# manhtuando97/two-stage-gnn

Hardware: NVIDIA B200
Metric: train graphs/sec (fwd+bwd) (higher is better)
Workload: dtype f32

## Files before the change

### include/tsg.h

```cpp
#ifndef TSG_H_
#define TSG_H_

#include <stddef.h>
#include <stdint.h>

#ifdef __cplusplus
extern "C" {
#endif

#define TSG_ABI_VERSION 1

enum {
  TSG_OK = 0,
  TSG_EINVAL = -1,
  TSG_EWORKSPACE = -2,
  TSG_ELAUNCH = -3,
  TSG_EARCH = -4
};

int tsg_abi_version(void);
const char* tsg_last_error(void);
int tsg_check_device(void);
int tsg_init_device(void);

// ... 190 lines not shown
int tsg_linkpred_loss_fwd(const float* S, const int64_t* graph_ptr, const int32_t* rowptr, const int32_t* colidx,
                          int64_t num_graphs, int64_t assign_dim, double num_entries, float eps, float* loss,
                          void* workspace, size_t workspace_bytes, void* stream);
int tsg_linkpred_loss_bwd(const float* S, const int64_t* graph_ptr, const int32_t* rowptr, const int32_t* colidx,
                          int64_t num_graphs, int64_t assign_dim, double num_entries, float eps, const float* dloss,
                          float* dS, void* stream);

#define TSG_TU_NETWORKX 0
#define TSG_TU_PYG 1
typedef struct tsg_tu_handle tsg_tu_handle;
int tsg_tu_load(const char* prefix, int mode, int64_t max_nodes , tsg_tu_handle** out);
int tsg_tu_sizes(const tsg_tu_handle* h, int64_t* sizes);
int tsg_tu_fill(const tsg_tu_handle* h, int64_t* node_ptr, int64_t* edge_ptr, int64_t* row, int64_t* col,
                int32_t* node_label, int64_t* y, float* attr );
void tsg_tu_free(tsg_tu_handle* h);

int tsg_csr_build_graphs_sym_local(const int32_t* local_row, const int32_t* local_col, const int64_t* edge_ptr,
                                   const int64_t* node_ptr, int64_t num_graphs, int64_t num_nodes, int64_t num_edges,
                                   int64_t max_graph_nodes, int32_t* rowptr, int32_t* colidx, float* val,
                                   int32_t* status, void* stream);

typedef struct {
  int64_t num_graphs, in_feat, hidden, num_edges;
  int64_t n[4];
  int64_t max_graph_nodes[3];
  int64_t max_graph_edges;
  double pooling_ratio;
  int64_t flags;
  int32_t* status;
} tsg_sag_shape;
#define TSG_SAG_COALESCED 1
size_t tsg_sag_arena_bytes(const tsg_sag_shape* shape);
int tsg_sag_set_fused(int on);
enum { TSG_SAG_PERM = 0, TSG_SAG_SCORE = 1, TSG_SAG_H = 2, TSG_SAG_XG = 3, TSG_SAG_ROWPTR = 4, TSG_SAG_COLIDX = 5,
       TSG_SAG_VAL = 6, TSG_SAG_INV = 7, TSG_SAG_STATUS = 8  };
int tsg_sag_arena_locate(const tsg_sag_shape* shape, int level, int field, size_t* offset, size_t* bytes);
int tsg_sag_encoder_fwd(const tsg_sag_shape* shape, const float* x, const int64_t* row, const int64_t* col,
                        const int64_t* level_ptr, const float* const* params, float* z,
                        void* arena, size_t arena_bytes, void* stream);
int tsg_sag_encoder_bwd(const tsg_sag_shape* shape, const float* x, const int64_t* level_ptr,
                        const float* const* params, const float* dz, float* const* grads,
                        void* arena, size_t arena_bytes, void* stream);

typedef struct {
  int64_t num_classes;
  int64_t num_triplets;
  float margin, eps, dropout_p;
  uint64_t seed;
} tsg_sag_head;
size_t tsg_sag_triplet_step_workspace_bytes(const tsg_sag_shape* shape, const tsg_sag_head* head);
int tsg_sag_triplet_step_compact(const tsg_sag_shape* shape, const tsg_sag_head* head, const int32_t* label,
                                 const int32_t* local_row, const int32_t* local_col, const int64_t* edge_ptr,
                                 const int64_t* level_ptr, const float* const* params, const int64_t* triplets,
                                 const float* dropout_mask , float* const* grads, float* loss,
                                 float* emb_out , void* arena, size_t arena_bytes, void* workspace,
                                 size_t workspace_bytes, void* stream);

int tsg_sag_step_fwd_compact(const tsg_sag_shape* shape, const tsg_sag_head* head, const int32_t* label,
                             const int32_t* local_row, const int32_t* local_col, const int64_t* edge_ptr,
                             const int64_t* level_ptr, const float* const* params, const float* dropout_mask ,
                             float* emb, void* arena, size_t arena_bytes, void* workspace, size_t workspace_bytes,
                             void* stream);
int tsg_sag_step_bwd_compact(const tsg_sag_shape* shape, const tsg_sag_head* head, const int32_t* label,
                             const int64_t* level_ptr, const float* const* params, const float* emb, const float* demb,
                             float* const* grads, void* arena, size_t arena_bytes, void* workspace,
                             size_t workspace_bytes, void* stream);
// ... 50 lines not shown
```

### two-stage-gnn_b200/csrc/k10_sag_exec.cu

```cuda
#include "common.cuh"
#include "sag_fused.cuh"

namespace tsg {

struct LevelBuf {
  int64_t* eptr;
  int32_t *rowptr, *colidx, *t_rowptr, *t_colidx;
  float *val, *t_val;
  float *xw, *h, *sw, *score, *xg, *out;
  int64_t* perm;
  int32_t* inv;
  int32_t* argmax;
};

struct SagArena {
  LevelBuf lv[3];
  float *dxg, *dh, *dhm, *dxw, *dscore, *dsw;
  void* scratch; size_t scratch_bytes;
  unsigned* sched; int* status;
  size_t total;
};

static size_t scratch_need(const tsg_sag_shape* sh) {
  size_t m = 0;
  auto up = [&](size_t v) { if (v > m) m = v; };
  for (int l = 0; l < 3; ++l) {
    up(tsg_csr_build_graphs_workspace_bytes(sh->num_graphs, sh->num_edges));
    up(tsg_topk_workspace_bytes(sh->n[l], sh->num_graphs));
    up(tsg_csr_filter_workspace_bytes(sh->n[l + 1]));
    up(2 * tsg_colsum_workspace_bytes(sh->n[l], sh->hidden));
    up(tsg_linear_bwd_weight_workspace_bytes(l == 0 ? sh->in_feat : sh->hidden, sh->hidden));
    up(tsg_linear_bwd_weight_workspace_bytes(sh->hidden, 1));
  }
  up(tsg_embed_bwd_weight_workspace_bytes(sh->in_feat, sh->hidden));
  up(tsg_gate_score_bwd_workspace_bytes());
  return align_up(m, 256) + 256;
}

static void layout(const tsg_sag_shape* sh, void* arena, SagArena* a) {
  char* base = (char*)arena;
  size_t off = 0;
  auto take = [&](size_t bytes) -> void* {
    void* p = base ? (void*)(base + off) : nullptr;
    off += align_up(bytes, 256);
    return p;
  };
  const int64_t G = sh->num_graphs, H = sh->hidden, E = sh->num_edges;
  for (int l = 0; l < 3; ++l) {
    LevelBuf& b = a->lv[l];
    const int64_t n = sh->n[l], k = sh->n[l + 1], cap = E + n;
    b.eptr = (int64_t*)take((G + 1) * 8);
    b.rowptr = (int32_t*)take((n + 1) * 4); b.t_rowptr = (int32_t*)take((n + 1) * 4);
    b.colidx = (int32_t*)take(cap * 4); b.t_colidx = (int32_t*)take(cap * 4);
    b.val = (float*)take(cap * 4); b.t_val = (float*)take(cap * 4);
    b.xw = (float*)take(n * H * 4); b.h = (float*)take(n * H * 4);
    b.sw = (float*)take(n * 4); b.score = (float*)take(n * 4);
    b.perm = (int64_t*)take((k > 0 ? k : 1) * 8);
    b.inv = (int32_t*)take((n > 0 ? n : 1) * 4);
    b.xg = (float*)take((k > 0 ? k : 1) * H * 4);
    b.out = (float*)take(G * 2 * H * 4);
    b.argmax = (int32_t*)take(G * H * 4);
  }
  const int64_t n0 = sh->n[0] > 0 ? sh->n[0] : 1;
  a->dxg = (float*)take(n0 * H * 4); a->dh = (float*)take(n0 * H * 4);
  a->dhm = (float*)take(n0 * H * 4); a->dxw = (float*)take(n0 * H * 4);
  a->dscore = (float*)take(n0 * 4); a->dsw = (float*)take(n0 * 4);
// ... 5 lines not shown
  a->total = off;
  if (sh->flags & TSG_SAG_COALESCED)
    for (int l = 0; l < 3; ++l) {
      LevelBuf& b = a->lv[l];
      b.t_rowptr = b.rowptr; b.t_colidx = b.colidx; b.t_val = b.val;
    }
}

__global__ void __launch_bounds__(256)
k_add3(const float* __restrict__ a, const float* __restrict__ b, const float* __restrict__ c, float* __restrict__ o, int64_t n) {
  for (int64_t i = (int64_t)blockIdx.x * blockDim.x + threadIdx.x; i < n; i += (int64_t)gridDim.x * blockDim.x)
    o[i] = (a[i] + b[i]) + c[i];
}

struct SagInput {
  const float* x;
  const int64_t *row, *col;
  const int32_t* label;
  const int32_t *lrow, *lcol;
  const int64_t* edge_ptr;
};

static bool sag_unfused_env() {
  static const bool v = getenv("TSG_SAG_UNFUSED") != nullptr;
  return v;
}

static int g_sag_fused = -1;
static bool sag_fused_env() {
  if (g_sag_fused < 0) g_sag_fused = !(getenv("TSG_SAG_FUSED") && getenv("TSG_SAG_FUSED")[0] == '0');
  return g_sag_fused != 0;
}

static bool use_fused(const tsg_sag_shape* sh, bool compact) {
  if (!compact || !sag_fused_env() || sh->max_graph_edges <= 0) return false;
  for (int l = 0; l < 3; ++l) if (sh->max_graph_nodes[l] > 32767) return false;
  return fused_supported((int)sh->hidden, (int)sh->in_feat, (int)sh->max_graph_nodes[0], (int)sh->max_graph_nodes[1],
                         (int)sh->max_graph_edges);
}

static void fill_fused(FusedArgs& f, const tsg_sag_shape* sh, const SagArena& a, const int32_t* label, const int32_t* lrow,
                       const int32_t* lcol, const int64_t* edge_ptr, const int64_t* level_ptr, const float* const* params) {
  f.G = (int)sh->num_graphs; f.L = (int)sh->in_feat; f.H = (int)sh->hidden;
  for (int l = 0; l < 3; ++l) f.nmax[l] = (int)sh->max_graph_nodes[l];
  f.emax = (int)sh->max_graph_edges;
  f.ratio = (float)sh->pooling_ratio; f.avg_degree = (double)sh->num_edges / (double)(sh->n[0] > 0 ? sh->n[0] : 1);
  f.cls = 0; f.cls_nlo = 0; f.cls_elo = -1;
  f.label = label; f.lrow = lrow; f.lcol = lcol; f.edge_ptr = edge_ptr; f.level_ptr = level_ptr;
  for (int i = 0; i < 12; ++i) f.params[i] = params[i];
  for (int l = 0; l < 3; ++l) {
    f.h[l] = a.lv[l].h; f.score[l] = a.lv[l].score; f.perm[l] = a.lv[l].perm; f.argmax[l] = a.lv[l].argmax;
  }
  f.z = nullptr;
  f.sched = a.sched; f.status = a.status;
}

static bool shape_ok(const tsg_sag_shape* sh) {
  if (!sh || sh->num_graphs <= 0 || sh->in_feat <= 0 || sh->hidden <= 0 || sh->num_edges < 0) return false;
  for (int l = 0; l < 4; ++l) if (sh->n[l] <= 0) return false;
  for (int l = 0; l < 3; ++l) if (sh->max_graph_nodes[l] <= 0) return false;
  return true;
}

}

using namespace tsg;

#define TSG_TRY(call)                 \
  do {                                \
    int _rc = (call);                 \
    if (_rc != TSG_OK) return _rc;    \
  } while (0)

extern "C" int tsg_sag_set_fused(int on) {
  const int prev = sag_fused_env() ? 1 : 0;
  g_sag_fused = on ? 1 : 0;
  return prev;
}

extern "C" size_t tsg_sag_arena_bytes(const tsg_sag_shape* shape) {
  if (!shape_ok(shape)) return 0;
  SagArena a;
  layout(shape, nullptr, &a);
  return a.total;
}

extern "C" int tsg_sag_arena_locate(const tsg_sag_shape* sh, int level, int field, size_t* offset, size_t* bytes) {
  TSG_REQUIRE(shape_ok(sh) && level >= 0 && level < 3 && offset && bytes, "sag_arena_locate: bad argument");
  SagArena a;
  char* const base = (char*)256;
  tsg_sag_shape own = *sh;
  own.status = nullptr;
  layout(&own, base, &a);
  const LevelBuf& b = a.lv[level];
  const int64_t n = sh->n[level], k = sh->n[level + 1], H = sh->hidden;
  const void* p = nullptr; size_t sz = 0;
  switch (field) {
    case TSG_SAG_PERM: p = b.perm; sz = (size_t)k * 8; break;
    case TSG_SAG_SCORE: p = b.score; sz = (size_t)n * 4; break;
    case TSG_SAG_H: p = b.h; sz = (size_t)n * H * 4; break;
    case TSG_SAG_XG: p = b.xg; sz = (size_t)k * H * 4; break;
    case TSG_SAG_ROWPTR: p = b.rowptr; sz = (size_t)(n + 1) * 4; break;
    case TSG_SAG_COLIDX: p = b.colidx; sz = (size_t)(sh->num_edges + n) * 4; break;
    case TSG_SAG_VAL: p = b.val; sz = (size_t)(sh->num_edges + n) * 4; break;
    case TSG_SAG_INV: p = b.inv; sz = (size_t)n * 4; break;
    case TSG_SAG_STATUS: p = a.status; sz = 4; break;
    default: set_error("sag_arena_locate: unknown field %d", field); return TSG_EINVAL;
  }
  *offset = (size_t)((const char*)p - base);
  *bytes = sz;
  return TSG_OK;
}

static int sag_fwd(const tsg_sag_shape* sh, const SagInput& in, const int64_t* level_ptr, const float* const* params,
                   float* z, void* arena, size_t arena_bytes, void* stream, bool forward_only = false) {
  SagArena a;
  layout(sh, arena, &a);
  if (arena_bytes < a.total) { set_error("sag_encoder_fwd: arena too small (%zu < %zu)", arena_bytes, a.total); return TSG_EWORKSPACE; }
  cudaStream_t st = (cudaStream_t)stream;
  const int64_t G = sh->num_graphs, H = sh->hidden, E = sh->num_edges;
  if (!sh->status) cudaMemsetAsync(a.status, 0, sizeof(int), st);
  if (forward_only && use_fused(sh, in.label != nullptr)) {
    FusedArgs f;
    fill_fused(f, sh, a, in.label, in.lrow, in.lcol, in.edge_ptr, level_ptr, params);
    f.z = z;
    return launch_sag_fused_fwd(f, st);
  }
  const float* xin = in.x;
  bool xw_ready = false;
  for (int l = 0; l < 3; ++l) {
    LevelBuf& b = a.lv[l];
    const int64_t n = sh->n[l], k = sh->n[l + 1], fin = l == 0 ? sh->in_feat : H;
    const float *W = params[4 * l], *bias = params[4 * l + 1], *ws = params[4 * l + 2], *bs = params[4 * l + 3];
    const int64_t* ptr_l = level_ptr + (size_t)l * (G + 1);
    const int64_t* ptr_n = level_ptr + (size_t)(l + 1) * (G + 1);
    const bool sym = in.label && (sh->flags & TSG_SAG_COALESCED);
    if (l == 0 && sym) {
      TSG_TRY(tsg_csr_build_graphs_sym_local(in.lrow, in.lcol, in.edge_ptr, ptr_l, G, n, E, sh->max_graph_nodes[l], b.rowptr,
                                             b.colidx, b.val, a.status, stream));
    } else if (l == 0 && in.label) {
      TSG_TRY(tsg_csr_build_graphs_local(in.lrow, in.lcol, in.edge_ptr, ptr_l, G, n, E, sh->max_graph_nodes[l], b.rowptr,
                                         b.colidx, b.val, nullptr, b.t_rowptr, b.t_colidx, b.t_val, nullptr, a.scratch,
                                         a.scratch_bytes, stream));
    } else if (l == 0) {
      TSG_TRY(tsg_edge_ptr(in.row, E, nullptr, ptr_l, G, b.eptr, stream));
      TSG_TRY(tsg_csr_build_graphs(in.row, in.col, b.eptr, ptr_l, G, n, E, sh->max_graph_nodes[l], b.rowptr, b.colidx, b.val,
                                   nullptr, b.t_rowptr, b.t_colidx, b.t_val, nullptr, a.scratch, a.scratch_bytes, stream));
    } else {
      const LevelBuf& pb = a.lv[l - 1];
      if (sym) TSG_TRY(tsg_csr_filter(pb.rowptr, pb.colidx, nullptr, nullptr, pb.perm, pb.inv, n, b.rowptr, b.colidx, b.val,
                                      nullptr, nullptr, nullptr, a.scratch, a.scratch_bytes, stream));
      else TSG_TRY(tsg_csr_filter(pb.rowptr, pb.colidx, pb.t_rowptr, pb.t_colidx, pb.perm, pb.inv, n, b.rowptr, b.colidx, b.val,
                                  b.t_rowptr, b.t_colidx, b.t_val, a.scratch, a.scratch_bytes, stream));
    }
    static const bool no_label_spmm = getenv("TSG_NO_LABEL_SPMM") != nullptr;
    const bool label_spmm = l == 0 && in.label && H % 4 == 0 && H <= 128 && !no_label_spmm &&
                            ((((uintptr_t)W) | ((uintptr_t)bias) | ((uintptr_t)ws)) & 15) == 0;
    if (label_spmm) {
      TSG_TRY(tsg_spmm_label_dot(b.rowptr, b.colidx, b.val, W, in.label, fin, bias, b.h, ws, b.sw, n, H, TSG_SPMM_RELU, stream));
    } else {
      if (l == 0 && in.label) TSG_TRY(tsg_embed_fwd(W, in.label, b.xw, n, fin, H, stream));
      else if (!xw_ready) TSG_TRY(tsg_linear_fwd(xin, W, nullptr, b.xw, n, fin, H, 0, 0, stream));
      TSG_TRY(tsg_spmm_dot(b.rowptr, b.colidx, b.val, b.xw, bias, b.h, ws, b.sw, n, H, TSG_SPMM_RELU, stream));
    }
    TSG_TRY(tsg_spmm(b.rowptr, b.colidx, b.val, b.sw, bs, b.score, n, 1, 0, stream));
    TSG_TRY(tsg_topk_bounded(b.score, ptr_l, ptr_n, G, n, sh->max_graph_nodes[l], b.perm, a.scratch, a.scratch_bytes, stream));
    TSG_TRY(tsg_inv_perm(b.perm, k, n, b.inv, stream));
    static const bool no_gr = getenv("TSG_NO_GATE_READOUT") != nullptr;
    if (H % 4 == 0 && !sag_unfused_env() && !no_gr) {
      const bool next_xw = l < 2 && (((uintptr_t)params[4 * (l + 1)]) & 15) == 0;
      TSG_TRY(tsg_gate_readout_linear_fwd(b.h, b.score, b.perm, ptr_n, G, k, H, b.xg, b.out, 2 * H, b.argmax,
                                          next_xw ? params[4 * (l + 1)] : nullptr, next_xw ? a.lv[l + 1].xw : nullptr, stream));
      xw_ready = next_xw;
    } else {
      xw_ready = false;
      TSG_TRY(tsg_gate_gather_fwd(b.h, b.score, b.perm, nullptr, b.xg, nullptr, k, H, stream));
      TSG_TRY(tsg_readout_fwd(b.xg, ptr_n, G, H, TSG_READOUT_MAX | TSG_READOUT_MEAN, b.out, 2 * H, b.argmax, stream));
    }
    xin = b.xg;
  }
  const int64_t tot = G * 2 * H;
  k_add3<<<grid_for(tot, 256, 8), 256, 0, st>>>(a.lv[0].out, a.lv[1].out, a.lv[2].out, z, tot);
  return check_launch("sag_encoder_fwd");
}

extern "C" int tsg_sag_encoder_fwd(const tsg_sag_shape* sh, const float* x, const int64_t* row, const int64_t* col,
                                   const int64_t* level_ptr, const float* const* params, float* z,
                                   void* arena, size_t arena_bytes, void* stream) {
  TSG_REQUIRE(shape_ok(sh), "sag_encoder_fwd: bad shape");
  TSG_REQUIRE(x && level_ptr && params && z && arena && (sh->num_edges == 0 || (row && col)), "sag_encoder_fwd: null pointer");
  const SagInput in{x, row, col, nullptr, nullptr, nullptr, nullptr};
  return sag_fwd(sh, in, level_ptr, params, z, arena, arena_bytes, stream);
}

extern "C" int tsg_sag_encoder_fwd_compact(const tsg_sag_shape* sh, const int32_t* label, const int32_t* local_row,
                                           const int32_t* local_col, const int64_t* edge_ptr, const int64_t* level_ptr,
                                           const float* const* params, float* z, void* arena, size_t arena_bytes,
                                           void* stream) {
  TSG_REQUIRE(shape_ok(sh), "sag_encoder_fwd_compact: bad shape");
  TSG_REQUIRE(label && edge_ptr && level_ptr && params && z && arena && (sh->num_edges == 0 || (local_row && local_col)),
// ... 79 lines not shown
```

### two-stage-gnn_b200/csrc/k5_topk.cu

```cuda
#include "common.cuh"
#include <stdlib.h>

namespace tsg {

__device__ __forceinline__ uint32_t score_key(float s) {
  if (s != s) return 0xFFFFFFFFu;
  if (s == 0.f) s = 0.f;
  uint32_t b = __float_as_uint(s);
  return (b & 0x80000000u) ? ~b : (b | 0x80000000u);
}

struct KofN {
  const int64_t* gptr; float ratio;
  __device__ int operator()(int64_t g) const {
    float n = (float)(gptr[g + 1] - gptr[g]);
    return (int)ceilf(__fmul_rn(ratio, n));
  }
};

constexpr int TOPK_THREADS = 128;
constexpr int TOPK_SMEM_KEYS = 4096;

__global__ void __launch_bounds__(TOPK_THREADS)
k_topk_rank(const float* __restrict__ score, const int64_t* __restrict__ gptr,
            const int64_t* __restrict__ kptr, int64_t* __restrict__ perm, unsigned long long* __restrict__ gkeys,
            int skip_upto) {
  __shared__ __align__(16) unsigned long long skeys[TOPK_SMEM_KEYS];
  const int g = blockIdx.x;
  const int64_t base = gptr[g];
  const int n = (int)(gptr[g + 1] - base);
  const int64_t obase = kptr[g];
  const int k = (int)(kptr[g + 1] - obase);
  if (n == 0 || k == 0) return;
  if (n <= skip_upto) return;
  const bool in_smem = n <= TOPK_SMEM_KEYS;
  unsigned long long* keys = in_smem ? skeys : (gkeys + base);
  for (int i = threadIdx.x; i < n; i += TOPK_THREADS)
    keys[i] = ((unsigned long long)score_key(score[base + i]) << 32) | (unsigned long long)(0xFFFFFFFFu - (unsigned)i);
  __syncthreads();
  for (int i = threadIdx.x; i < n; i += TOPK_THREADS) {
    const unsigned long long ki = keys[i];
    int rank = 0;
    int j = 0;
// ... 12 lines not shown
            int64_t* __restrict__ perm, int max_pad, int min_n) {
  extern __shared__ __align__(16) unsigned long long sk[];
  {
    const int g = blockIdx.x;
    const int64_t base = gptr[g];
    const int n = (int)(gptr[g + 1] - base);
    const int64_t obase = kptr[g];
    const int k = (int)(kptr[g + 1] - obase);
    if (n == 0 || k == 0) return;
    if (n > max_pad) return;
    if (n <= min_n) return;
    int npad = 32; while (npad < n) npad <<= 1;
    for (int i = threadIdx.x; i < npad; i += TOPK_SORT_THREADS)
      sk[i] = i < n ? (((unsigned long long)score_key(score[base + i]) << 32) | (unsigned long long)(0xFFFFFFFFu - (unsigned)i)) : 0ull;
    __syncthreads();
    for (int kk = 2; kk <= npad; kk <<= 1) {
      for (int j = kk >> 1; j > 0; j >>= 1) {
        for (int t = threadIdx.x; t < (npad >> 1); t += TOPK_SORT_THREADS) {
          const int i = ((t & ~(j - 1)) << 1) | (t & (j - 1));
          const int l = i | j;
          const unsigned long long a = sk[i], b = sk[l];
          const bool desc = (i & kk) == 0;
          if ((a < b) == desc) { sk[i] = b; sk[l] = a; }
        }
        __syncthreads();
      }
    }
    for (int i = threadIdx.x; i < k; i += TOPK_SORT_THREADS)
      perm[obase + i] = base + (int64_t)(0xFFFFFFFFu - (unsigned)(sk[i] & 0xFFFFFFFFull));
  }
}


constexpr int TOPK_RUN_THREADS = 256;
template <int KPT>
__device__ __forceinline__ void topk_runs_body(const float* __restrict__ score, int64_t base, int n, int k,
                                               int64_t obase, int64_t* __restrict__ perm, unsigned long long* runs) {
  constexpr int NW = TOPK_RUN_THREADS / 32, RL = 32 * KPT;
  const int lane = threadIdx.x & 31, w = threadIdx.x >> 5;
  unsigned long long key[KPT];
#pragma unroll
  for (int s = 0; s < KPT; ++s) {
    const int i = w * RL + s * 32 + lane;
    key[s] = i < n ? (((unsigned long long)score_key(score[base + i]) << 32) | (unsigned long long)(0xFFFFFFFFu - (unsigned)i)) : 0ull;
  }
#pragma unroll
  for (int kk = 2; kk <= RL; kk <<= 1) {
#pragma unroll
    for (int j = kk >> 1; j > 0; j >>= 1) {
      if (j >= 32) {
        const int js = j >> 5;
#pragma unroll
        for (int s = 0; s < KPT; ++s) {
          if ((s & js) == 0) {
            const bool desc = ((s * 32 + lane) & kk) == 0;
            const unsigned long long x = key[s], y = key[s | js];
            if ((x < y) == desc) { key[s] = y; key[s | js] = x; }
          }
        }
      } else {
#pragma unroll
        for (int s = 0; s < KPT; ++s) {
          const unsigned long long x = key[s];
          const unsigned long long y = __shfl_xor_sync(0xffffffffu, x, j);
          const bool keep_max = ((lane & j) == 0) == ((((s * 32 + lane) & kk)) == 0);
          key[s] = keep_max ? (x > y ? x : y) : (x < y ? x : y);
        }
      }
    }
  }
#pragma unroll
  for (int s = 0; s < KPT; ++s) runs[w * RL + s * 32 + lane] = key[s];
  __syncthreads();
#pragma unroll
  for (int s = 0; s < KPT; ++s) {
    const unsigned long long x = key[s];
    if (x == 0ull) continue;
    int rank = s * 32 + lane;
    for (int r = 0; r < NW && r * RL < n; ++r) {
      if (r == w) continue;
      const unsigned long long* run = runs + r * RL;
      int lo = 0, hi = RL;
      while (lo < hi) {
        const int mid = (lo + hi) >> 1;
        if (run[mid] > x) lo = mid + 1; else hi = mid;
      }
      rank += lo;
    }
    if (rank < k) perm[obase + rank] = base + (int64_t)(0xFFFFFFFFu - (unsigned)(x & 0xFFFFFFFFull));
  }
}

template <int KPT>
__device__ __forceinline__ void topk_warp_body(const float* __restrict__ score, int64_t base, int n, int k,
                                               int64_t obase, int64_t* __restrict__ perm) {
  constexpr int RL = 32 * KPT;
  const int lane = threadIdx.x & 31;
  unsigned long long key[KPT];
#pragma unroll
  for (int s = 0; s < KPT; ++s) {
    const int i = s * 32 + lane;
    key[s] = i < n ? (((unsigned long long)score_key(score[base + i]) << 32) | (unsigned long long)(0xFFFFFFFFu - (unsigned)i)) : 0ull;
  }
#pragma unroll
  for (int kk = 2; kk <= RL; kk <<= 1) {
#pragma unroll
    for (int j = kk >> 1; j > 0; j >>= 1) {
      if (j >= 32) {
        const int js = j >> 5;
#pragma unroll
        for (int s = 0; s < KPT; ++s) {
          if ((s & js) == 0) {
            const bool desc = ((s * 32 + lane) & kk) == 0;
            const unsigned long long x = key[s], y = key[s | js];
            if ((x < y) == desc) { key[s] = y; key[s | js] = x; }
          }
        }
      } else {
#pragma unroll
        for (int s = 0; s < KPT; ++s) {
          const unsigned long long x = key[s];
          const unsigned long long y = __shfl_xor_sync(0xffffffffu, x, j);
          const bool keep_max = ((lane & j) == 0) == ((((s * 32 + lane) & kk)) == 0);
          key[s] = keep_max ? (x > y ? x : y) : (x < y ? x : y);
        }
      }
    }
  }
#pragma unroll
  for (int s = 0; s < KPT; ++s) {
    const int rank = s * 32 + lane;
    if (key[s] != 0ull && rank < k) perm[obase + rank] = base + (int64_t)(0xFFFFFFFFu - (unsigned)(key[s] & 0xFFFFFFFFull));
  }
}

constexpr int TOPK_WARP_KEYS = 128;

__global__ void __launch_bounds__(TOPK_RUN_THREADS)
k_topk_runs(const float* __restrict__ score, const int64_t* __restrict__ gptr, const int64_t* __restrict__ kptr,
            int64_t* __restrict__ perm, int G, int cta_blocks) {
  __shared__ __align__(16) unsigned long long runs[TOPK_RUN_THREADS * 4];
  constexpr int NW = TOPK_RUN_THREADS / 32;
  if ((int)blockIdx.x >= cta_blocks) {
    const int nwarps = ((int)gridDim.x - cta_blocks) * NW;
    for (int g = ((int)blockIdx.x - cta_blocks) * NW + (threadIdx.x >> 5); g < G; g += nwarps) {
      const int64_t base = gptr[g];
      const int n = (int)(gptr[g + 1] - base);
      if (n <= 0 || n > TOPK_WARP_KEYS) continue;
      const int64_t obase = kptr[g];
      const int k = (int)(kptr[g + 1] - obase);
      if (k <= 0) continue;
      if (n <= 32) topk_warp_body<1>(score, base, n, k, obase, perm);
      else if (n <= 64) topk_warp_body<2>(score, base, n, k, obase, perm);
      else topk_warp_body<4>(score, base, n, k, obase, perm);
    }
    return;
  }
  for (int g = blockIdx.x; g < G; g += cta_blocks) {
    const int64_t base = gptr[g];
    const int n = (int)(gptr[g + 1] - base);
    if (n <= TOPK_WARP_KEYS || n > TOPK_RUN_THREADS * 4) continue;
    const int64_t obase = kptr[g];
    const int k = (int)(kptr[g + 1] - obase);
    if (k > 0) {
      if (n <= TOPK_RUN_THREADS) topk_runs_body<1>(score, base, n, k, obase, perm, runs);
      else if (n <= 2 * TOPK_RUN_THREADS) topk_runs_body<2>(score, base, n, k, obase, perm, runs);
      else topk_runs_body<4>(score, base, n, k, obase, perm, runs);
    }
    __syncthreads();
  }
}

__global__ void k_batch_to_ptr(const int64_t* __restrict__ batch, int64_t n, int64_t G, int64_t* __restrict__ gptr) {
  for (int64_t i = (int64_t)blockIdx.x * blockDim.x + threadIdx.x; i <= n;
       i += (int64_t)gridDim.x * blockDim.x) {
    int64_t prev = i == 0 ? -1 : batch[i - 1];
    int64_t cur = i == n ? G : batch[i];
    if (cur > G) cur = G;
    for (int64_t g = prev + 1; g <= cur; ++g) gptr[g] = i;
  }
}

constexpr int FA_THREADS = 256;
constexpr int FA_ITEMS = 8;
constexpr int FA_TILE = FA_THREADS * FA_ITEMS;

__global__ void k_inv_perm(const int64_t* __restrict__ perm, int64_t k, int* __restrict__ inv) {
  for (int64_t i = (int64_t)blockIdx.x * blockDim.x + threadIdx.x; i < k;
       i += (int64_t)gridDim.x * blockDim.x)
    inv[perm[i]] = (int)i;
}

template <bool WRITE>
__global__ void __launch_bounds__(FA_THREADS)
k_filter_adj(const int64_t* __restrict__ row, const int64_t* __restrict__ col, int64_t E_cap,
             const int64_t* __restrict__ E_dev, const int* __restrict__ inv,
             int* __restrict__ tile_cnt, const int* __restrict__ tile_off,
             int64_t* __restrict__ out_row, int64_t* __restrict__ out_col) {
  __shared__ int wcnt[FA_ITEMS][FA_THREADS / 32];
  __shared__ int woff[FA_ITEMS][FA_THREADS / 32];
// ... 342 lines not shown
```

### two-stage-gnn_b200/csrc/sag_fused.cuh

```cuda
#pragma once
#include "common.cuh"

namespace tsg {

struct FusedArgs {
  int G, L, H;
  int nmax[3];
  int emax;
  float ratio; double avg_degree;
  int cls, cls_nlo, cls_elo;
  const int32_t* label; const int32_t* lrow; const int32_t* lcol;
  const int64_t* edge_ptr;
  const int64_t* level_ptr;
  const float* params[12];
  float* h[3]; float* score[3]; int64_t* perm[3]; int32_t* argmax[3];
  float* z;
  unsigned* sched;
  int* status;
};

enum { TSG_FUSED_BAD_EDGE = 1, TSG_FUSED_UNSORTED = 2, TSG_FUSED_ASYMMETRIC = 4 };

bool fused_supported(int H, int L, int nmax0, int nmax1, int emax);
int fused_num_ctas();
int launch_sag_fused_fwd(const FusedArgs& a, cudaStream_t st);

}
```

### two-stage-gnn_b200/tsg/_lib.py

```python
from __future__ import annotations

import ctypes
import os
from ctypes import c_char_p, c_float, c_int, c_int64, c_size_t, c_void_p

import torch

_HERE = os.path.dirname(os.path.abspath(__file__))
LIB_PATH = os.path.join(os.path.dirname(_HERE), "libtsg.so")

P, I64, SZ, I, F32 = c_void_p, c_int64, c_size_t, c_int, c_float

_PROTOTYPES = {
    "tsg_abi_version": (I, []),
    "tsg_last_error": (c_char_p, []),
    "tsg_check_device": (I, []),
    "tsg_init_device": (I, []),
    "tsg_pack_batch": (I, [P, P, P, I64, P, P, P, P, P, P, I64, P, P, P, P]),
    "tsg_pack_batch_compact": (I, [P, P, P, I64, P, P, P, P, P, P, P, P, P]),
    "tsg_csr_build_workspace_bytes": (SZ, [I64, I64]),
    "tsg_csr_build": (I, [P, P, P, I64, P, I64, I, P, P, P, P, P, P, P, P, P, SZ, P]),
    "tsg_edge_ptr": (I, [P, I64, P, P, I64, P, P]),
    "tsg_csr_build_graphs_workspace_bytes": (SZ, [I64, I64]),
    "tsg_csr_build_graphs": (I, [P, P, P, P, I64, I64, I64, I64, P, P, P, P, P, P, P, P, P, SZ, P]),
# ... 24 lines not shown
    "tsg_seg_linear": (I, [P, P, P, I64, I64, I64, I, P, P]),
    "tsg_seg_linear_tc": (I, [P, P, P, I64, I64, I64, I, P, P, P]),
    "tsg_linear_tc": (I, [P, P, P, I64, I64, I64, I, I, P, P, P]),
    "tsg_topk_workspace_bytes": (SZ, [I64, I64]),
    "tsg_topk_sizes": (I, [P, I64, F32, P, P, SZ, P]),
    "tsg_topk": (I, [P, P, P, I64, I64, P, P, SZ, P]),
    "tsg_topk_bounded": (I, [P, P, P, I64, I64, I64, P, P, SZ, P]),
    "tsg_batch_to_ptr": (I, [P, I64, I64, P, P]),
    "tsg_filter_adj_workspace_bytes": (SZ, [I64]),
    "tsg_filter_adj": (I, [P, P, I64, P, P, I64, I64, P, P, P, P, P, SZ, P]),
    "tsg_gate_gather_fwd": (I, [P, P, P, P, P, P, I64, I64, P]),
    "tsg_gate_gather_bwd": (I, [P, P, P, P, P, P, I64, I64, P]),
    "tsg_readout_fwd": (I, [P, P, I64, I64, I, P, I64, P, P]),
    "tsg_readout_bwd": (I, [P, I64, P, P, I64, I64, I64, I, P, P]),
    "tsg_triplet_workspace_bytes": (SZ, [I64, I64, I64]),
    "tsg_triplet_fwd": (I, [P, P, I64, I64, I64, F32, F32, P, P, P, P, SZ, P]),
    "tsg_triplet_bwd": (I, [P, P, I64, I64, I64, F32, F32, P, P, P, P, P, SZ, P]),
    "tsg_pairdist_matrix": (I, [P, I64, I64, F32, P, P]),
    "tsg_eigpool_build": (I, [P, P, P, P, P, P, I64, I64, I, P, P, P, P, P]),
    "tsg_coarsen_edges_workspace_bytes": (SZ, [I64]),
    "tsg_coarsen_edges": (I, [P, P, P, I64, P, P, P, P, P, P, SZ, P]),
    "tsg_linkpred_workspace_bytes": (SZ, [I64]),
    "tsg_linkpred_loss_fwd": (I, [P, P, P, P, I64, I64, ctypes.c_double, F32, P, P, SZ, P]),
    "tsg_linkpred_loss_bwd": (I, [P, P, P, P, I64, I64, ctypes.c_double, F32, P, P, P]),
    "tsg_knn_predict": (I, [P, P, P, I64, I64, I64, I, I, P, P]),
    "tsg_mlp1_train": (I, [P, P, I64, I64, I64, I64, I64, P, P, P, I64, F32, F32, F32, F32, F32, P, P]),
    "tsg_tu_load": (I, [c_char_p, I, I64, P]),
    "tsg_tu_sizes": (I, [P, P]),
    "tsg_tu_fill": (I, [P, P, P, P, P, P, P, P]),
    "tsg_tu_free": (None, [P]),
    "tsg_sag_arena_bytes": (SZ, [P]),
    "tsg_sag_arena_locate": (I, [P, I, I, P, P]),
    "tsg_sag_set_fused": (I, [I]),
    "tsg_sag_triplet_step_workspace_bytes": (SZ, [P, P]),
    "tsg_sag_triplet_step_compact": (I, [P, P, P, P, P, P, P, P, P, P, P, P, P, P, SZ, P, SZ, P]),
    "tsg_sag_step_fwd_compact": (I, [P, P, P, P, P, P, P, P, P, P, P, SZ, P, SZ, P]),
    "tsg_sag_step_bwd_compact": (I, [P, P, P, P, P, P, P, P, P, SZ, P, SZ, P]),
    "tsg_sag_encoder_fwd": (I, [P, P, P, P, P, P, P, P, SZ, P]),
    "tsg_sag_encoder_bwd": (I, [P, P, P, P, P, P, P, SZ, P]),
    "tsg_sag_encoder_fwd_compact": (I, [P, P, P, P, P, P, P, P, P, SZ, P]),
    "tsg_sag_encoder_bwd_compact": (I, [P, P, P, P, P, P, P, SZ, P]),
    "tsg_sag_encoder_embed_compact": (I, [P, P, P, P, P, P, P, P, P, SZ, P]),
    "tsg_gate_score_bwd_workspace_bytes": (SZ, []),
    "tsg_gate_score_bwd": (I, [P, P, P, P, I64, I64, I64, P, P, P, SZ, P]),
    "tsg_gate_readout_fwd": (I, [P, P, P, P, I64, I64, P, P, I64, P, P]),
    "tsg_gate_readout_linear_fwd": (I, [P, P, P, P, I64, I64, I64, P, P, I64, P, P, P, P]),
    "tsg_spmm_label_dot": (I, [P, P, P, P, P, I64, P, P, P, P, I64, I64, I, P]),
    "tsg_spmm_dot": (I, [P, P, P, P, P, P, P, P, I64, I64, I, P]),
    "tsg_sag_conv_bwd_fused": (I, [P, P, P, P, P, P, P, P, P, I64, I64, P, SZ, P]),
    "tsg_embed_fwd": (I, [P, P, P, I64, I64, I64, P]),
    "tsg_embed_bwd_weight_workspace_bytes": (SZ, [I64, I64]),
    "tsg_embed_bwd_weight": (I, [P, P, P, I64, I64, I64, P, SZ, P]),
}


class SagShape(ctypes.Structure):
    _fields_ = [("num_graphs", c_int64), ("in_feat", c_int64), ("hidden", c_int64), ("num_edges", c_int64),
                ("n", c_int64 * 4), ("max_graph_nodes", c_int64 * 3), ("max_graph_edges", c_int64), ("pooling_ratio", ctypes.c_double), ("flags", c_int64), ("status", c_void_p)]

class SagHead(ctypes.Structure):
    _fields_ = [("num_classes", c_int64), ("num_triplets", c_int64), ("margin", c_float), ("eps", c_float),
                ("dropout_p", c_float), ("seed", ctypes.c_uint64)]


EXPORTS = tuple(_PROTOTYPES)

# ... 76 lines not shown
```

Measured before the change: 2.556 million.

## Fuse per-level top-k, inverse permutation and next-level CSR filtering

Adds a level-select path that does the per-graph top-k, writes the inverse permutation, and counts surviving neighbours in one kernel. A second kernel then builds the next level's normalized CSR using a decoupled look-back scan, replacing the separate topk, inv_perm and csr_filter launches. The top-k sort bodies move to a shared header and take an emit callback. This cuts kernel launches and intermediate passes, at the cost of a spin-waiting look-back scan that depends on blocks being scheduled in ticket order.

```diff
diff --git a/include/tsg.h b/include/tsg.h
--- a/include/tsg.h
+++ b/include/tsg.h
@@ -246,6 +246,7 @@
 #define TSG_SAG_COALESCED 1
 size_t tsg_sag_arena_bytes(const tsg_sag_shape* shape);
 int tsg_sag_set_fused(int on);
+int tsg_sag_set_level_select(int on);
 enum { TSG_SAG_PERM = 0, TSG_SAG_SCORE = 1, TSG_SAG_H = 2, TSG_SAG_XG = 3, TSG_SAG_ROWPTR = 4, TSG_SAG_COLIDX = 5,
        TSG_SAG_VAL = 6, TSG_SAG_INV = 7, TSG_SAG_STATUS = 8  };
 int tsg_sag_arena_locate(const tsg_sag_shape* shape, int level, int field, size_t* offset, size_t* bytes);
diff --git a/two-stage-gnn_b200/csrc/k10_sag_exec.cu b/two-stage-gnn_b200/csrc/k10_sag_exec.cu
--- a/two-stage-gnn_b200/csrc/k10_sag_exec.cu
+++ b/two-stage-gnn_b200/csrc/k10_sag_exec.cu
@@ -32,6 +32,7 @@
     up(tsg_linear_bwd_weight_workspace_bytes(l == 0 ? sh->in_feat : sh->hidden, sh->hidden));
     up(tsg_linear_bwd_weight_workspace_bytes(sh->hidden, 1));
   }
+  for (int l = 0; l < 3; ++l) up(level_select_workspace_bytes(sh->n[l + 1]));
   up(tsg_embed_bwd_weight_workspace_bytes(sh->in_feat, sh->hidden));
   up(tsg_gate_score_bwd_workspace_bytes());
   return align_up(m, 256) + 256;
@@ -103,6 +104,12 @@
   return g_sag_fused != 0;
 }
 
+static int g_level_select = -1;
+static bool level_select_env() {
+  if (g_level_select < 0) g_level_select = !(getenv("TSG_LEVEL_SELECT") && getenv("TSG_LEVEL_SELECT")[0] == '0');
+  return g_level_select != 0;
+}
+
 static bool use_fused(const tsg_sag_shape* sh, bool compact) {
   if (!compact || !sag_fused_env() || sh->max_graph_edges <= 0) return false;
   for (int l = 0; l < 3; ++l) if (sh->max_graph_nodes[l] > 32767) return false;
@@ -146,6 +153,12 @@
 extern "C" int tsg_sag_set_fused(int on) {
   const int prev = sag_fused_env() ? 1 : 0;
   g_sag_fused = on ? 1 : 0;
+  return prev;
+}
+
+extern "C" int tsg_sag_set_level_select(int on) {
+  const int prev = level_select_env() ? 1 : 0;
+  g_level_select = on ? 1 : 0;
   return prev;
 }
 
@@ -199,6 +212,7 @@
   }
   const float* xin = in.x;
   bool xw_ready = false;
+  bool csr_ready = false;
   for (int l = 0; l < 3; ++l) {
     LevelBuf& b = a.lv[l];
     const int64_t n = sh->n[l], k = sh->n[l + 1], fin = l == 0 ? sh->in_feat : H;
@@ -217,7 +231,7 @@
       TSG_TRY(tsg_edge_ptr(in.row, E, nullptr, ptr_l, G, b.eptr, stream));
       TSG_TRY(tsg_csr_build_graphs(in.row, in.col, b.eptr, ptr_l, G, n, E, sh->max_graph_nodes[l], b.rowptr, b.colidx, b.val,
                                    nullptr, b.t_rowptr, b.t_colidx, b.t_val, nullptr, a.scratch, a.scratch_bytes, stream));
-    } else {
+    } else if (!csr_ready) {
       const LevelBuf& pb = a.lv[l - 1];
       if (sym) TSG_TRY(tsg_csr_filter(pb.rowptr, pb.colidx, nullptr, nullptr, pb.perm, pb.inv, n, b.rowptr, b.colidx, b.val,
                                       nullptr, nullptr, nullptr, a.scratch, a.scratch_bytes, stream));
@@ -235,8 +249,21 @@
       TSG_TRY(tsg_spmm_dot(b.rowptr, b.colidx, b.val, b.xw, bias, b.h, ws, b.sw, n, H, TSG_SPMM_RELU, stream));
     }
     TSG_TRY(tsg_spmm(b.rowptr, b.colidx, b.val, b.sw, bs, b.score, n, 1, 0, stream));
-    TSG_TRY(tsg_topk_bounded(b.score, ptr_l, ptr_n, G, n, sh->max_graph_nodes[l], b.perm, a.scratch, a.scratch_bytes, stream));
-    TSG_TRY(tsg_inv_perm(b.perm, k, n, b.inv, stream));
+    const bool select = sym && level_select_env() && sh->max_graph_nodes[l] <= LEVEL_SELECT_MAX_NODES;
+    if (select) {
+      LevelSelectArgs s;
+      s.rowptr = b.rowptr; s.colidx = b.colidx; s.score = b.score;
+      s.node_ptr = ptr_l; s.k_ptr = ptr_n; s.G = (int)G; s.n = n; s.k = k;
+      s.perm = b.perm; s.inv = b.inv;
+      LevelBuf* nx = l < 2 ? &a.lv[l + 1] : nullptr;
+      s.next_rowptr = nx ? nx->rowptr : nullptr; s.next_colidx = nx ? nx->colidx : nullptr;
+      s.next_val = nx ? nx->val : nullptr;
+      TSG_TRY(launch_level_select(s, a.scratch, a.scratch_bytes, st));
+    } else {
+      TSG_TRY(tsg_topk_bounded(b.score, ptr_l, ptr_n, G, n, sh->max_graph_nodes[l], b.perm, a.scratch, a.scratch_bytes, stream));
+      TSG_TRY(tsg_inv_perm(b.perm, k, n, b.inv, stream));
+    }
+    csr_ready = select && l < 2;
     static const bool no_gr = getenv("TSG_NO_GATE_READOUT") != nullptr;
     if (H % 4 == 0 && !sag_unfused_env() && !no_gr) {
       const bool next_xw = l < 2 && (((uintptr_t)params[4 * (l + 1)]) & 15) == 0;
diff --git a/two-stage-gnn_b200/csrc/k16_level_select.cu b/two-stage-gnn_b200/csrc/k16_level_select.cu
--- /dev/null
+++ b/two-stage-gnn_b200/csrc/k16_level_select.cu
@@ -0,0 +1,152 @@
+#include "common.cuh"
+#include "sag_fused.cuh"
+#include "topk_runs.cuh"
+
+namespace tsg {
+
+constexpr int LS_THREADS = TOPK_RUN_THREADS;
+constexpr int LS_WARPS = LS_THREADS / 32;
+constexpr int LS_ROWS = LS_THREADS;
+
+constexpr unsigned long long LS_AGGREGATE = 1ull << 62, LS_INCLUSIVE = 1ull << 63, LS_VALUE = (1ull << 62) - 1;
+
+__device__ __forceinline__ int ls_count_row(const int32_t* __restrict__ rowptr, const int32_t* __restrict__ colidx,
+                                            const int32_t* inv, int64_t r) {
+  int c = 0;
+  for (int p = __ldg(rowptr + r), e = __ldg(rowptr + r + 1); p < e; ++p) c += inv[__ldg(colidx + p)] >= 0;
+  return c;
+}
+
+__global__ void __launch_bounds__(LS_THREADS, 5)
+k_sel_topk_count(const float* __restrict__ score, const int64_t* __restrict__ gptr, const int64_t* __restrict__ kptr,
+                 int64_t* perm, int32_t* inv, const int32_t* __restrict__ rowptr, const int32_t* __restrict__ colidx,
+                 int32_t* __restrict__ cnt, int G, int cta_blocks, unsigned long long* __restrict__ zero, int zero_n) {
+  __shared__ __align__(16) unsigned long long runs[TOPK_RUN_THREADS * 4];
+  for (int i = blockIdx.x * LS_THREADS + threadIdx.x; i < zero_n; i += gridDim.x * LS_THREADS) zero[i] = 0ull;
+  const int lane = threadIdx.x & 31;
+  if ((int)blockIdx.x >= cta_blocks) {
+    const int nwarps = ((int)gridDim.x - cta_blocks) * LS_WARPS;
+    for (int g = ((int)blockIdx.x - cta_blocks) * LS_WARPS + (threadIdx.x >> 5); g < G; g += nwarps) {
+      const int64_t base = gptr[g];
+      const int n = (int)(gptr[g + 1] - base);
+      if (n <= 0 || n > TOPK_WARP_KEYS) continue;
+      const int64_t obase = kptr[g];
+      const int k = (int)(kptr[g + 1] - obase);
+      auto emit = [=](int rank, int i) {
+        inv[base + i] = rank < k ? (int)(obase + rank) : -1;
+        if (rank < k) perm[obase + rank] = base + i;
+      };
+      if (n <= 32) topk_warp_body<1>(score + base, n, emit);
+      else if (n <= 64) topk_warp_body<2>(score + base, n, emit);
+      else topk_warp_body<4>(score + base, n, emit);
+      if (!cnt) continue;
+      __syncwarp();
+      for (int i = lane; i < k; i += 32) cnt[obase + i] = ls_count_row(rowptr, colidx, inv, perm[obase + i]);
+    }
+    return;
+  }
+  for (int g = blockIdx.x; g < G; g += cta_blocks) {
+    const int64_t base = gptr[g];
+    const int n = (int)(gptr[g + 1] - base);
+    if (n <= TOPK_WARP_KEYS || n > TOPK_RUN_THREADS * 4) continue;
+    const int64_t obase = kptr[g];
+    const int k = (int)(kptr[g + 1] - obase);
+    auto emit = [=](int rank, int i) {
+      inv[base + i] = rank < k ? (int)(obase + rank) : -1;
+      if (rank < k) perm[obase + rank] = base + i;
+    };
+    if (n <= TOPK_RUN_THREADS) topk_runs_body<1>(score + base, n, runs, emit);
+    else if (n <= 2 * TOPK_RUN_THREADS) topk_runs_body<2>(score + base, n, runs, emit);
+    else topk_runs_body<4>(score + base, n, runs, emit);
+    __syncthreads();
+    if (cnt)
+      for (int i = threadIdx.x; i < k; i += LS_THREADS) cnt[obase + i] = ls_count_row(rowptr, colidx, inv, perm[obase + i]);
+  }
+}
+
+__device__ int ls_lookback(unsigned long long* status, int t, int count) {
+  const int lane = threadIdx.x & 31;
+  if (t == 0) {
+    if (lane == 0) atomicExch(status, LS_INCLUSIVE | (unsigned long long)count);
+    return 0;
+  }
+  if (lane == 0) atomicExch(status + t, LS_AGGREGATE | (unsigned long long)count);
+  long long excl = 0;
+  for (int end = t;; end -= 32) {
+    const int j = end - 1 - lane;
+    unsigned long long s = LS_INCLUSIVE;
+    if (j >= 0)
+      do { s = *(volatile unsigned long long*)(status + j); } while (s == 0);
+    const unsigned inc = __ballot_sync(0xffffffffu, (s & LS_INCLUSIVE) != 0);
+    const int stop = inc ? __ffs(inc) - 1 : 31;
+    long long v = lane <= stop ? (long long)(s & LS_VALUE) : 0;
+#pragma unroll
+    for (int d = 16; d > 0; d >>= 1) v += __shfl_xor_sync(0xffffffffu, v, d);
+    excl += v;
+    if (inc) break;
+  }
+  if (lane == 0) atomicExch(status + t, LS_INCLUSIVE | (unsigned long long)(excl + count));
+  return (int)excl;
+}
+
+__global__ void __launch_bounds__(LS_THREADS)
+k_sel_csr_write(const int32_t* __restrict__ rowptr, const int32_t* __restrict__ colidx, const int64_t* __restrict__ perm,
+                const int32_t* __restrict__ inv, const int32_t* __restrict__ cnt, int K, unsigned long long* status,
+                int items, int32_t* __restrict__ n_rowptr, int32_t* __restrict__ n_colidx, float* __restrict__ n_val) {
+  __shared__ int sm[33];
+  __shared__ int s_t, s_excl;
+  if (threadIdx.x == 0) s_t = (int)atomicAdd(reinterpret_cast<unsigned*>(status + items), 1u);
+  __syncthreads();
+  const int t = s_t;
+  const int i = t * LS_ROWS + threadIdx.x;
+  const int c = i < K ? __ldg(cnt + i) : 0;
+  int total;
+  const int ex = block_excl_scan(c, sm, &total);
+  if (threadIdx.x < 32) {
+    const int e = ls_lookback(status, t, total);
+    if (threadIdx.x == 0) s_excl = e;
+  }
+  __syncthreads();
+  if (i >= K) return;
+  int o = s_excl + ex;
+  n_rowptr[i] = o;
+  if (i == K - 1) n_rowptr[K] = o + c;
+  const float dr = __fdiv_rn(1.0f, __fsqrt_rn((float)c));
+  const int64_t r = __ldg(perm + i);
+  for (int p = __ldg(rowptr + r), e = __ldg(rowptr + r + 1); p < e; ++p) {
+    const int j = __ldg(inv + __ldg(colidx + p));
+    if (j < 0) continue;
+    const float dj = __fdiv_rn(1.0f, __fsqrt_rn((float)__ldg(cnt + j)));
+    n_colidx[o] = j;
+    n_val[o] = __fmul_rn(__fmul_rn(dj, 1.0f), dr);
+    ++o;
+  }
+}
+
+static int ls_items(int64_t k) { return (int)((k + LS_ROWS - 1) / LS_ROWS); }
+
+size_t level_select_workspace_bytes(int64_t k) {
+  return ws_bytes((size_t)k + 1, 4) + ws_bytes((size_t)ls_items(k) + 1, 8);
+}
+
+int launch_level_select(const LevelSelectArgs& a, void* workspace, size_t workspace_bytes, cudaStream_t st) {
+  TSG_REQUIRE(a.G > 0 && a.n > 0 && a.k > 0 && a.k < (int64_t)0x3fffffff, "level_select: bad sizes");
+  const bool csr = a.next_rowptr != nullptr;
+  if (csr && workspace_bytes < level_select_workspace_bytes(a.k)) { set_error("level_select: workspace too small"); return TSG_EWORKSPACE; }
+  Workspace ws(workspace, workspace_bytes);
+  int32_t* cnt = csr ? ws.take<int32_t>((size_t)a.k + 1) : nullptr;
+  const int items = ls_items(a.k);
+  unsigned long long* status = csr ? ws.take<unsigned long long>((size_t)items + 1) : nullptr;
+  const int G = a.G;
+  const int cta_blocks = G < TSG_NUM_SMS * 8 ? G : TSG_NUM_SMS * 8;
+  const int groups = (G + LS_WARPS - 1) / LS_WARPS;
+  const int warp_blocks = groups < TSG_NUM_SMS * 4 ? groups : TSG_NUM_SMS * 4;
+  k_sel_topk_count<<<cta_blocks + warp_blocks, LS_THREADS, 0, st>>>(a.score, a.node_ptr, a.k_ptr, a.perm, a.inv, a.rowptr,
+                                                                  a.colidx, cnt, G, cta_blocks, status, csr ? items + 1 : 0);
+  if (csr)
+    k_sel_csr_write<<<items, LS_THREADS, 0, st>>>(a.rowptr, a.colidx, a.perm, a.inv, cnt, (int)a.k, status, items,
+                                                   a.next_rowptr, a.next_colidx, a.next_val);
+  return check_launch("level_select");
+}
+
+}
diff --git a/two-stage-gnn_b200/csrc/k5_topk.cu b/two-stage-gnn_b200/csrc/k5_topk.cu
--- a/two-stage-gnn_b200/csrc/k5_topk.cu
+++ b/two-stage-gnn_b200/csrc/k5_topk.cu
@@ -1,14 +1,8 @@
 #include "common.cuh"
+#include "topk_runs.cuh"
 #include <stdlib.h>
 
 namespace tsg {
-
-__device__ __forceinline__ uint32_t score_key(float s) {
-  if (s != s) return 0xFFFFFFFFu;
-  if (s == 0.f) s = 0.f;
-  uint32_t b = __float_as_uint(s);
-  return (b & 0x80000000u) ? ~b : (b | 0x80000000u);
-}
 
 struct KofN {
   const int64_t* gptr; float ratio;
@@ -87,109 +81,6 @@
 }
 
 
-constexpr int TOPK_RUN_THREADS = 256;
-template <int KPT>
-__device__ __forceinline__ void topk_runs_body(const float* __restrict__ score, int64_t base, int n, int k,
-                                               int64_t obase, int64_t* __restrict__ perm, unsigned long long* runs) {
-  constexpr int NW = TOPK_RUN_THREADS / 32, RL = 32 * KPT;
-  const int lane = threadIdx.x & 31, w = threadIdx.x >> 5;
-  unsigned long long key[KPT];
-#pragma unroll
-  for (int s = 0; s < KPT; ++s) {
-    const int i = w * RL + s * 32 + lane;
-    key[s] = i < n ? (((unsigned long long)score_key(score[base + i]) << 32) | (unsigned long long)(0xFFFFFFFFu - (unsigned)i)) : 0ull;
-  }
-#pragma unroll
-  for (int kk = 2; kk <= RL; kk <<= 1) {
-#pragma unroll
-    for (int j = kk >> 1; j > 0; j >>= 1) {
-      if (j >= 32) {
-        const int js = j >> 5;
-#pragma unroll
-        for (int s = 0; s < KPT; ++s) {
-          if ((s & js) == 0) {
-            const bool desc = ((s * 32 + lane) & kk) == 0;
-            const unsigned long long x = key[s], y = key[s | js];
-            if ((x < y) == desc) { key[s] = y; key[s | js] = x; }
-          }
-        }
-      } else {
-#pragma unroll
-        for (int s = 0; s < KPT; ++s) {
-          const unsigned long long x = key[s];
-          const unsigned long long y = __shfl_xor_sync(0xffffffffu, x, j);
-          const bool keep_max = ((lane & j) == 0) == ((((s * 32 + lane) & kk)) == 0);
-          key[s] = keep_max ? (x > y ? x : y) : (x < y ? x : y);
-        }
-      }
-    }
-  }
-#pragma unroll
-  for (int s = 0; s < KPT; ++s) runs[w * RL + s * 32 + lane] = key[s];
-  __syncthreads();
-#pragma unroll
-  for (int s = 0; s < KPT; ++s) {
-    const unsigned long long x = key[s];
-    if (x == 0ull) continue;
-    int rank = s * 32 + lane;
-    for (int r = 0; r < NW && r * RL < n; ++r) {
-      if (r == w) continue;
-      const unsigned long long* run = runs + r * RL;
-      int lo = 0, hi = RL;
-      while (lo < hi) {
-        const int mid = (lo + hi) >> 1;
-        if (run[mid] > x) lo = mid + 1; else hi = mid;
-      }
-      rank += lo;
-    }
-    if (rank < k) perm[obase + rank] = base + (int64_t)(0xFFFFFFFFu - (unsigned)(x & 0xFFFFFFFFull));
-  }
-}
-
-template <int KPT>
-__device__ __forceinline__ void topk_warp_body(const float* __restrict__ score, int64_t base, int n, int k,
-                                               int64_t obase, int64_t* __restrict__ perm) {
-  constexpr int RL = 32 * KPT;
-  const int lane = threadIdx.x & 31;
-  unsigned long long key[KPT];
-#pragma unroll
-  for (int s = 0; s < KPT; ++s) {
-    const int i = s * 32 + lane;
-    key[s] = i < n ? (((unsigned long long)score_key(score[base + i]) << 32) | (unsigned long long)(0xFFFFFFFFu - (unsigned)i)) : 0ull;
-  }
-#pragma unroll
-  for (int kk = 2; kk <= RL; kk <<= 1) {
-#pragma unroll
-    for (int j = kk >> 1; j > 0; j >>= 1) {
-      if (j >= 32) {
-        const int js = j >> 5;
-#pragma unroll
-        for (int s = 0; s < KPT; ++s) {
-          if ((s & js) == 0) {
-            const bool desc = ((s * 32 + lane) & kk) == 0;
-            const unsigned long long x = key[s], y = key[s | js];
-            if ((x < y) == desc) { key[s] = y; key[s | js] = x; }
-          }
-        }
-      } else {
-#pragma unroll
-        for (int s = 0; s < KPT; ++s) {
-          const unsigned long long x = key[s];
-          const unsigned long long y = __shfl_xor_sync(0xffffffffu, x, j);
-          const bool keep_max = ((lane & j) == 0) == ((((s * 32 + lane) & kk)) == 0);
-          key[s] = keep_max ? (x > y ? x : y) : (x < y ? x : y);
-        }
-      }
-    }
-  }
-#pragma unroll
-  for (int s = 0; s < KPT; ++s) {
-    const int rank = s * 32 + lane;
-    if (key[s] != 0ull && rank < k) perm[obase + rank] = base + (int64_t)(0xFFFFFFFFu - (unsigned)(key[s] & 0xFFFFFFFFull));
-  }
-}
-
-constexpr int TOPK_WARP_KEYS = 128;
 
 __global__ void __launch_bounds__(TOPK_RUN_THREADS)
 k_topk_runs(const float* __restrict__ score, const int64_t* __restrict__ gptr, const int64_t* __restrict__ kptr,
@@ -205,9 +96,10 @@
       const int64_t obase = kptr[g];
       const int k = (int)(kptr[g + 1] - obase);
       if (k <= 0) continue;
-      if (n <= 32) topk_warp_body<1>(score, base, n, k, obase, perm);
-      else if (n <= 64) topk_warp_body<2>(score, base, n, k, obase, perm);
-      else topk_warp_body<4>(score, base, n, k, obase, perm);
+      auto emit = [&](int rank, int i) { if (rank < k) perm[obase + rank] = base + i; };
+      if (n <= 32) topk_warp_body<1>(score + base, n, emit);
+      else if (n <= 64) topk_warp_body<2>(score + base, n, emit);
+      else topk_warp_body<4>(score + base, n, emit);
     }
     return;
   }
@@ -218,9 +110,10 @@
     const int64_t obase = kptr[g];
     const int k = (int)(kptr[g + 1] - obase);
     if (k > 0) {
-      if (n <= TOPK_RUN_THREADS) topk_runs_body<1>(score, base, n, k, obase, perm, runs);
-      else if (n <= 2 * TOPK_RUN_THREADS) topk_runs_body<2>(score, base, n, k, obase, perm, runs);
-      else topk_runs_body<4>(score, base, n, k, obase, perm, runs);
+      auto emit = [&](int rank, int i) { if (rank < k) perm[obase + rank] = base + i; };
+      if (n <= TOPK_RUN_THREADS) topk_runs_body<1>(score + base, n, runs, emit);
+      else if (n <= 2 * TOPK_RUN_THREADS) topk_runs_body<2>(score + base, n, runs, emit);
+      else topk_runs_body<4>(score + base, n, runs, emit);
     }
     __syncthreads();
   }
diff --git a/two-stage-gnn_b200/csrc/sag_fused.cuh b/two-stage-gnn_b200/csrc/sag_fused.cuh
--- a/two-stage-gnn_b200/csrc/sag_fused.cuh
+++ b/two-stage-gnn_b200/csrc/sag_fused.cuh
@@ -25,4 +25,16 @@
 int fused_num_ctas();
 int launch_sag_fused_fwd(const FusedArgs& a, cudaStream_t st);
 
+constexpr int LEVEL_SELECT_MAX_NODES = 1024;
+struct LevelSelectArgs {
+  const int32_t *rowptr, *colidx;
+  const float* score;
+  const int64_t *node_ptr, *k_ptr;
+  int G; int64_t n, k;
+  int64_t* perm; int32_t* inv;
+  int32_t *next_rowptr, *next_colidx; float* next_val;
+};
+size_t level_select_workspace_bytes(int64_t n);
+int launch_level_select(const LevelSelectArgs& a, void* workspace, size_t workspace_bytes, cudaStream_t st);
+
 }
diff --git a/two-stage-gnn_b200/csrc/topk_runs.cuh b/two-stage-gnn_b200/csrc/topk_runs.cuh
--- /dev/null
+++ b/two-stage-gnn_b200/csrc/topk_runs.cuh
@@ -0,0 +1,122 @@
+#pragma once
+#include "common.cuh"
+
+namespace tsg {
+
+__device__ __forceinline__ uint32_t score_key(float s) {
+  if (s != s) return 0xFFFFFFFFu;
+  if (s == 0.f) s = 0.f;
+  uint32_t b = __float_as_uint(s);
+  return (b & 0x80000000u) ? ~b : (b | 0x80000000u);
+}
+
+__device__ __forceinline__ unsigned long long topk_key(float s, int i) {
+  return ((unsigned long long)score_key(s) << 32) | (unsigned long long)(0xFFFFFFFFu - (unsigned)i);
+}
+
+__device__ __forceinline__ int topk_key_index(unsigned long long key) {
+  return (int)(0xFFFFFFFFu - (unsigned)(key & 0xFFFFFFFFull));
+}
+
+constexpr int TOPK_RUN_THREADS = 256;
+template <int KPT, typename Emit>
+__device__ __forceinline__ void topk_runs_body(const float* score, int n, unsigned long long* runs, Emit emit) {
+  constexpr int NW = TOPK_RUN_THREADS / 32, RL = 32 * KPT;
+  const int lane = threadIdx.x & 31, w = threadIdx.x >> 5;
+  unsigned long long key[KPT];
+#pragma unroll
+  for (int s = 0; s < KPT; ++s) {
+    const int i = w * RL + s * 32 + lane;
+    key[s] = i < n ? topk_key(score[i], i) : 0ull;
+  }
+#pragma unroll
+  for (int kk = 2; kk <= RL; kk <<= 1) {
+#pragma unroll
+    for (int j = kk >> 1; j > 0; j >>= 1) {
+      if (j >= 32) {
+        const int js = j >> 5;
+#pragma unroll
+        for (int s = 0; s < KPT; ++s) {
+          if ((s & js) == 0) {
+            const bool desc = ((s * 32 + lane) & kk) == 0;
+            const unsigned long long x = key[s], y = key[s | js];
+            if ((x < y) == desc) { key[s] = y; key[s | js] = x; }
+          }
+        }
+      } else {
+#pragma unroll
+        for (int s = 0; s < KPT; ++s) {
+          const unsigned long long x = key[s];
+          const unsigned long long y = __shfl_xor_sync(0xffffffffu, x, j);
+          const bool keep_max = ((lane & j) == 0) == ((((s * 32 + lane) & kk)) == 0);
+          key[s] = keep_max ? (x > y ? x : y) : (x < y ? x : y);
+        }
+      }
+    }
+  }
+#pragma unroll
+  for (int s = 0; s < KPT; ++s) runs[w * RL + s * 32 + lane] = key[s];
+  __syncthreads();
+#pragma unroll
+  for (int s = 0; s < KPT; ++s) {
+    const unsigned long long x = key[s];
+    if (x == 0ull) continue;
+    int rank = s * 32 + lane;
+    for (int r = 0; r < NW && r * RL < n; ++r) {
+      if (r == w) continue;
+      const unsigned long long* run = runs + r * RL;
+      int lo = 0, hi = RL;
+      while (lo < hi) {
+        const int mid = (lo + hi) >> 1;
+        if (run[mid] > x) lo = mid + 1; else hi = mid;
+      }
+      rank += lo;
+    }
+    emit(rank, topk_key_index(x));
+  }
+}
+
+constexpr int TOPK_WARP_KEYS = 128;
+template <int KPT, typename Emit>
+__device__ __forceinline__ void topk_warp_body(const float* score, int n, Emit emit) {
+  constexpr int RL = 32 * KPT;
+  const int lane = threadIdx.x & 31;
+  unsigned long long key[KPT];
+#pragma unroll
+  for (int s = 0; s < KPT; ++s) {
+    const int i = s * 32 + lane;
+    key[s] = i < n ? topk_key(score[i], i) : 0ull;
+  }
+#pragma unroll
+  for (int kk = 2; kk <= RL; kk <<= 1) {
+#pragma unroll
+    for (int j = kk >> 1; j > 0; j >>= 1) {
+      if (j >= 32) {
+        const int js = j >> 5;
+#pragma unroll
+        for (int s = 0; s < KPT; ++s) {
+          if ((s & js) == 0) {
+            const bool desc = ((s * 32 + lane) & kk) == 0;
+            const unsigned long long x = key[s], y = key[s | js];
+            if ((x < y) == desc) { key[s] = y; key[s | js] = x; }
+          }
+        }
+      } else {
+#pragma unroll
+        for (int s = 0; s < KPT; ++s) {
+          const unsigned long long x = key[s];
+          const unsigned long long y = __shfl_xor_sync(0xffffffffu, x, j);
+          const bool keep_max = ((lane & j) == 0) == ((((s * 32 + lane) & kk)) == 0);
+          key[s] = keep_max ? (x > y ? x : y) : (x < y ? x : y);
+        }
+      }
+    }
+  }
+#pragma unroll
+  for (int s = 0; s < KPT; ++s) {
+    const int rank = s * 32 + lane;
+    if (key[s] != 0ull) emit(rank, topk_key_index(key[s]));
+  }
+}
+
+}
diff --git a/two-stage-gnn_b200/tsg/_lib.py b/two-stage-gnn_b200/tsg/_lib.py
--- a/two-stage-gnn_b200/tsg/_lib.py
+++ b/two-stage-gnn_b200/tsg/_lib.py
@@ -80,6 +80,7 @@
     "tsg_sag_arena_bytes": (SZ, [P]),
     "tsg_sag_arena_locate": (I, [P, I, I, P, P]),
     "tsg_sag_set_fused": (I, [I]),
+    "tsg_sag_set_level_select": (I, [I]),
     "tsg_sag_triplet_step_workspace_bytes": (SZ, [P, P]),
     "tsg_sag_triplet_step_compact": (I, [P, P, P, P, P, P, P, P, P, P, P, P, P, P, SZ, P, SZ, P]),
     "tsg_sag_step_fwd_compact": (I, [P, P, P, P, P, P, P, P, P, P, P, SZ, P, SZ, P]),
```

New measurement: 2.644 million (median of 6 runs). 1.03x the previous value.
